# bruno-maruszczak/lap-time-optimization

Measured on AMD Instinct MI355X. Metric: MPC solves/sec (N=40, nx=8 [7 + progress s], nu=2), higher is better.
Workload: dtype f64

## Files before the change

### lap-time-optimization_amd/csrc/layout.h

```cpp
#pragma once
#include "model.h"

namespace ltompc {


constexpr int FILTER_MAX = 16;
constexpr double DW_KEEP = 1e-5;
constexpr int MAX_LS = 12;
constexpr double ELASTIC_CP_VIOL = 0.1;
constexpr double RHO_UNIT = 1000.0;
__host__ __device__ __forceinline__ double pen_scale(const double rho) { return rho > RHO_UNIT ? rho / RHO_UNIT : 1.0; }

enum : int {
  QP_A = 0,
  QP_B = 64,
  QP_b = 80,
  QP_Q = 88,
  QP_S = 124,
  QP_R = 140,
  QP_q0 = 143,
  QP_q1 = 151,
  QP_r0 = 159,
  QP_r1 = 161,
  QP_Qx = 163,
  QP_qx0 = 199,
  QP_qx1 = 207,
  QP_NF = 215
};
enum : int { RC_K = 0, RC_Kv = 16, RC_kff = 20, RC_P = 22, RC_Pxv = 58, RC_pp = 74, RC_NF = 82 };
enum : int { RS_rd = 0, RS_rp, RS_cmax, RS_cmin, RS_smult, RS_cost, RS_emax, RS_NF };
enum : int { SP_apri = 0, SP_adua, SP_gphid, SP_NF };
enum : int {
  ST_MU = 0, ST_EPS, ST_EPS_NEXT, ST_DW_LAST, ST_FORCE_REG, ST_ALPHA, ST_ADUA, ST_E0, ST_OBJ, ST_TAU,
  ST_THETA0, ST_THMAX, ST_THMIN, ST_DW, ST_DW_TRY,
  ST_C00,
  ST_RHO,
  ST_VIOL,
  ST_G0,
  ST_NF
};
enum : int { SI_STATUS = 0, SI_ITERS, SI_NACC, SI_NTINY, SI_NFILT, SI_DONE, SI_STEP, SI_NREG, SI_NLSFAIL, SI_RETRY, SI_TRIES,
             SI_SKIP_EVAL, SI_LSMORE, SI_PREV, SI_RESTO, SI_REINIT, SI_NRESTO,
             SI_STICKY,
             SI_STARTEL,
             SI_SWEEPS,
             SI_PHASE, SI_TICKS, SI_FINAL,
             SI_WARM,
             SI_SHIFT,
             SI_NSHIFT,
             SI_SINCEMU,
             SI_FBARMED,
             SI_NFALLBACK,
             SI_BLOWUP,
             SI_NODE0,
             SI_NF };

struct Work {
  int N, B, Bp;
  gptr<double> X, C, U, L1, L2, T, NU;
  gptr<double> dX, dC, dU, nL1, nL2, dT, dNU;
  gptr<double> QP, RC, RS, SP, LS;
  gptr<double> x0, uprev;
  gptr<double> st;
  gptr<double> filt;
  gptr<int> si;
  gptr<int> active;
  gptr<double> DBG;
  gptr<int> ls_list, ls_count;
  gptr<double> BK;
  gptr<const int> orig;
};

struct Launch {
  gptr<const int> act;
  gptr<const int> nact;
  int n_pad;
  int force_eval;
};

struct Consts {
  ltompc_params p;
  ltompc_options o;
  Tables T;
  Bounds bd;
};

#define PL(base, f, k, NK) ((base)[((size_t)(f) * (NK) + (k)) * W.Bp + b])
#define PG(base, f, k, NF) ((base)[(((size_t)(k) * (W.Bp >> 3) + (b >> 3)) * (NF) + (f)) * 8 + (b & 7)])


#define STD(f) st[(size_t)(f) * W.Bp + b]
#define STI(f) si[(size_t)(f) * W.Bp + b]

#define WAVE_SYNC()                                        \
  do {                                                     \
    __builtin_amdgcn_fence(__ATOMIC_RELEASE, "wavefront"); \
    __builtin_amdgcn_wave_barrier();                       \
    __builtin_amdgcn_fence(__ATOMIC_ACQUIRE, "wavefront"); \
  } while (0)

#if !defined(LTOMPC_HOST_HARNESS)
__device__ __forceinline__ double grp_max(double v) {
  v = fmax(v, __shfl_xor(v, 8)), v = fmax(v, __shfl_xor(v, 16)), v = fmax(v, __shfl_xor(v, 32));
  return v;
}
__device__ __forceinline__ double grp_sum(double v) {
  v += __shfl_xor(v, 8), v += __shfl_xor(v, 16), v += __shfl_xor(v, 32);
  return v;
}
__device__ __forceinline__ double grp_min(double v) {
  v = fmin(v, __shfl_xor(v, 8)), v = fmin(v, __shfl_xor(v, 16)), v = fmin(v, __shfl_xor(v, 32));
  return v;
}

#else
using ::grp_max;
using ::grp_min;
using ::grp_sum;
#endif

}
```

### lap-time-optimization_amd/csrc/linearise.h

```cpp
#pragma once
#include "layout.h"

namespace ltompc {

__device__ __forceinline__ double sym_get(const double* H, int i, int j) { return H[sidx(i, j)]; }


struct BoundsAny {
  static constexpr bool fixed = false;
  static constexpr unsigned ulb = 0, uub = 0, xlb = 0, xub = 0;
};
template <unsigned ULB, unsigned UUB, unsigned XLB, unsigned XUB>
struct BoundsFixed {
  static constexpr bool fixed = true;
  static constexpr unsigned ulb = ULB, uub = UUB, xlb = XLB, xub = XUB;
};
using BoundsRef = BoundsFixed<0x3, 0x3, 0xCD, 0xC4>;

template <class BP, typename F>
__device__ __forceinline__ int for_each_bound(const ltompc_params& p, F&& f) {
  int m = 0;
#pragma unroll
  for (int i = 0; i < 2; i++) {
    if (BP::fixed ? ((BP::ulb >> i) & 1u) != 0 : p.u_lb[i] > -LTOMPC_NO_BOUND) f(m++, 0, i, -1.0, p.u_lb[i]);
// ... 327 lines not shown
  if (COL < 8) {
#pragma unroll
    for (int i = 0; i <= RM; i++) v[i] = ((i == COL) ? 2.0 : 0.0) - ((COL >= elo_(i) && COL <= ehi_(i)) ? 4.0 * S.E2[i * 8 + COL] : 0.0);
  } else if (COL < 10) {
    constexpr int j = 6 + COL - 8;
#pragma unroll
    for (int i = 0; i < 8; i++) v[i] = -hdt * (((i == j) ? 1.0 : 0.0) + ((j >= elo_(i) && j <= ehi_(i)) ? 2.0 * S.E2[i * 8 + j] : 0.0));
  } else {
#pragma unroll
    for (int i = 0; i < 8; i++) {
      double s = -S.G2[i];
#pragma unroll
      for (int l = elo_(i); l <= ehi_(i); l++) s -= 2.0 * S.E2[i * 8 + l] * S.G1[l];
      v[i] = s;
    }
  }
  m8_solve<RM>(M, v, y);
#pragma unroll
  for (int i = 0; i <= RM; i++) Y[i * 11 + COL] = y[i];
#pragma unroll
  for (int i = 0; i < 8; i++) {
    double s;
    if (COL < 8) s = (i == COL) ? 2.0 : 0.0;
    else if (COL < 10) s = (i == 6 + COL - 8) ? hdt : 0.0;
    else s = S.G1[i];
#pragma unroll
    for (int l = elo_(i); l <= imin_(ehi_(i), RM); l++) s += S.E1[i * 8 + l] * y[l];
    AB[i * 11 + COL] = 2.0 * s;
  }
}

__device__ __forceinline__ bool factor_m8(const Slot& S, M8Blocks& M) {
  double maa[9], mbb[9];
#pragma unroll
  for (int i = 0; i < 6; i++)
#pragma unroll
    for (int j = gs_(i); j < 8; j++) {
      double s = (i == j) ? 4.5 : 0.0;
#pragma unroll
      for (int l = elo_(i); l <= imin_(ehi_(i), ge_(j)); l++)
        if (j >= elo_(l) && j <= ehi_(l)) s += 2.0 * S.E2[i * 8 + l] * S.E1[l * 8 + j];
      if (i < 3) {
        if (j < 3) maa[i * 3 + j] = s;
        else if (j < 6) M.ab[i * 3 + j - 3] = s;
        else M.ac[i * 2 + j - 6] = s;
      } else {
        if (j < 6) mbb[(i - 3) * 3 + j - 3] = s;
        else M.bc[(i - 3) * 2 + j - 6] = s;
      }
    }
  return inv33(maa, M.iaa) & inv33(mbb, M.ibb);
}

__device__ __forceinline__ bool condense_slot(const Consts& K, const Slot& S, M8Blocks& M, double* Y, double* AB) {
  const bool ok = factor_m8(S, M);
#pragma unroll
  for (int q = 0; q < 88; q++) Y[q] = 0.0, AB[q] = 0.0;
  condense_column<0>(K, S, M, Y, AB), condense_column<1>(K, S, M, Y, AB), condense_column<2>(K, S, M, Y, AB);
  condense_column<3>(K, S, M, Y, AB), condense_column<4>(K, S, M, Y, AB), condense_column<5>(K, S, M, Y, AB);
  condense_column<6>(K, S, M, Y, AB), condense_column<7>(K, S, M, Y, AB), condense_column<8>(K, S, M, Y, AB);
  condense_column<9>(K, S, M, Y, AB), condense_column<10>(K, S, M, Y, AB);
  return ok;
}


template <class BP, bool ELL>
__device__ __forceinline__ void d_eval(const Consts& K, const Work& W, const int k, const int b, const bool force) {
  const int N = W.N;
  if (W.si[(size_t)SI_DONE * W.Bp + b]) return;
  if (!force && (W.si[(size_t)SI_RETRY * W.Bp + b] || W.si[(size_t)SI_SKIP_EVAL * W.Bp + b])) return;
  const double hdt = K.o.t_step;
  const double eps = W.st[(size_t)ST_EPS * W.Bp + b];
  const bool reinit = W.si[(size_t)SI_REINIT * W.Bp + b] != 0;
  if (reinit) reinit_slot<BP>(K, W, k, b);
  Slot S;
  linearise_slot<true, BP, ELL>(K, W, k, b, eps, S);
#pragma unroll
  for (int i = 0; i < 36; i++) PG(W.QP, QP_Qx + i, k + 1, QP_NF) = S.Hxp[i];
#pragma unroll
  for (int i = 0; i < 8; i++) PG(W.QP, QP_qx0 + i, k + 1, QP_NF) = S.gxp0[i], PG(W.QP, QP_qx1 + i, k + 1, QP_NF) = S.gxp1[i];
  {
    double l1[8], l2[8], l1n[8], l2n[8], rd = 0.0, rp = 0.0, sm = 0.0;
    const int kn = k + 1 < N ? k + 1 : k;
    const bool nxt = k + 1 < N && !reinit;
#pragma unroll
    for (int i = 0; i < 8; i++) l1[i] = PL(W.L1, i, k, N), l2[i] = PL(W.L2, i, k, N), l1n[i] = PL(W.L1, i, kn, N), l2n[i] = PL(W.L2, i, kn, N);
#pragma unroll
    for (int a = 0; a < 8; a++) {
      double rcx = S.dcd[a] + 4.5 * l2[a];
      double rxp = S.dxd[a] - 0.5 * l1[a];
#pragma unroll
      for (int i = 0; i <= ge_(a); i++)
        if (a >= elo_(i) && a <= ehi_(i)) rcx += S.E1[i * 8 + a] * l1[i], rxp += S.E2[i * 8 + a] * l2[i];
      {
        const double t = 2.0 * l1n[a] - 2.0 * l2n[a];
        const double r2 = rxp + t;
        rxp = nxt ? r2 : rxp;
      }
      rd = fmax(rd, fmax(fabs(rcx), fabs(rxp)));
      rp = fmax(rp, fmax(fabs(S.G1[a]), fabs(S.G2[a])));
      sm += fabs(l1[a]) + fabs(l2[a]);
    }
    double cost = S.cost;
#pragma unroll
    for (int i = 0; i < 2; i++) {
      double v = k ? PL(W.U, i, k - 1, N) : W.uprev[(size_t)i * W.Bp + b];
      double du = S.u[i] - v;
      cost += K.p.r_du[i] * du * du;
      double ru = S.dud[i] + 2.0 * K.p.r_du[i] * du + hdt * (l1[6 + i] + l2[6 + i]);
      if (k + 1 < N) ru -= 2.0 * K.p.r_du[i] * (PL(W.U, i, k + 1, N) - S.u[i]);
      rd = fmax(rd, fabs(ru));
    }
    rp = fmax(rp, S.rp_ineq), sm += S.smult;
    const double cmax = S.cmax, cmin = S.cmin;
    double th0 = S.th_ineq;
#pragma unroll
    for (int a = 0; a < 8; a++) th0 += fabs(S.G1[a]) + fabs(S.G2[a]);
    PL(W.LS, 0, k, N) = th0, PL(W.LS, 1, k, N) = cost, PL(W.LS, 2, k, N) = S.sumlog;
    PL(W.RS, RS_rd, k, N) = rd, PL(W.RS, RS_rp, k, N) = rp, PL(W.RS, RS_cmax, k, N) = cmax;
    PL(W.RS, RS_cmin, k, N) = cmin, PL(W.RS, RS_smult, k, N) = sm, PL(W.RS, RS_cost, k, N) = cost;
    PL(W.RS, RS_emax, k, N) = S.emax;
  }
  M8Blocks M8;
  double Y[88], AB[88];
  condense_slot(K, S, M8, Y, AB);
#pragma unroll
  for (int i = 0; i < 8; i++) {
#pragma unroll
    for (int j = 0; j < 8; j++) PG(W.QP, QP_A + i * 8 + j, k, QP_NF) = AB[i * 11 + j];
    PG(W.QP, QP_B + i * 2 + 0, k, QP_NF) = AB[i * 11 + 8], PG(W.QP, QP_B + i * 2 + 1, k, QP_NF) = AB[i * 11 + 9];
    PG(W.QP, QP_b + i, k, QP_NF) = AB[i * 11 + 10];
  }
  double HY[88];
#pragma unroll
  for (int i = 0; i < 8; i++)
#pragma unroll
    for (int col = 0; col < 11; col++) {
      double s = 0.0;
#pragma unroll
      for (int l = 0; l <= yrow_(col); l++)
        if (hnz_(i, l)) s += sym_get(S.Hc, i, l) * Y[l * 11 + col];
      HY[i * 11 + col] = s;
    }
#pragma unroll
  for (int i = 0; i < 10; i++) {
#pragma unroll
    for (int j = 0; j < 10; j++) {
      if (j > i) continue;
      double s = 0.0;
#pragma unroll
      for (int l = 0; l <= yrow_(i); l++) s += Y[l * 11 + i] * HY[l * 11 + j];
      if (i < 8) PG(W.QP, QP_Q + sidx(i, j), k, QP_NF) = s;
      else if (j < 8) PG(W.QP, QP_S + (i - 8) * 8 + j, k, QP_NF) = s;
      else PG(W.QP, QP_R + sidx(i - 8, j - 8), k, QP_NF) = s + ((i == j) ? S.Du[i - 8] : 0.0);
    }
    double s0 = 0.0, s1 = 0.0;
#pragma unroll
    for (int l = 0; l <= yrow_(i); l++) s0 += Y[l * 11 + i] * (HY[l * 11 + 10] + S.gc0[l]), s1 += Y[l * 11 + i] * S.gc1[l];
    if (i < 8) PG(W.QP, QP_q0 + i, k, QP_NF) = s0, PG(W.QP, QP_q1 + i, k, QP_NF) = s1;
    else PG(W.QP, QP_r0 + i - 8, k, QP_NF) = s0 + S.gub0[i - 8], PG(W.QP, QP_r1 + i - 8, k, QP_NF) = s1 + S.gub1[i - 8];
  }
}

template <class BP, bool ELL>
__global__ void __launch_bounds__(64) k_eval(const Consts* __restrict__ Kp, const Work* __restrict__ Wp, Launch la) {
  const Consts& K = *Kp;
  const Work& W = *Wp;
  int tid = blockIdx.x * blockDim.x + threadIdx.x;
  int j = tid % la.n_pad, k = tid / la.n_pad;
  if (k >= W.N || j >= la.nact[0]) return;
  d_eval<BP, ELL>(K, W, k, la.act[j], la.force_eval != 0);
}


template <class BP, bool ELL>
__device__ __forceinline__ void d_expand(const Consts& K, const Work& W, const int k, const int b) {
  const int N = W.N;
  if (W.si[(size_t)SI_DONE * W.Bp + b] || !W.si[(size_t)SI_STEP * W.Bp + b]) return;
  const double mu = W.st[(size_t)ST_MU * W.Bp + b], eps = W.st[(size_t)ST_EPS * W.Bp + b];
  const double tau = W.st[(size_t)ST_TAU * W.Bp + b], rho = W.st[(size_t)ST_RHO * W.Bp + b];
  double pi[8];
  {
    double dxp0[8], du0[2];
#pragma unroll
    for (int i = 0; i < 8; i++) dxp0[i] = PL(W.dX, i, k + 1, N + 1);
    du0[0] = PL(W.dU, 0, k, N), du0[1] = PL(W.dU, 1, k, N);
#pragma unroll
    for (int i = 0; i < 8; i++) {
      double s = PG(W.RC, RC_pp + i, k + 1, RC_NF) + PG(W.RC, RC_Pxv + i * 2, k + 1, RC_NF) * du0[0] +
                 PG(W.RC, RC_Pxv + i * 2 + 1, k + 1, RC_NF) * du0[1];
#pragma unroll
      for (int j = 0; j < 8; j++) s += PG(W.RC, RC_P + sidx(i, j), k + 1, RC_NF) * dxp0[j];
      pi[i] = s;
    }
  }
  __builtin_amdgcn_sched_barrier(0);
  Slot S;
  linearise_slot<false, BP, ELL>(K, W, k, b, eps, S);
  M8Blocks M8;
  factor_m8(S, M8);
  double dxk[8], dxp[8], du[2], dc[8];
#pragma unroll
  for (int i = 0; i < 8; i++) dxk[i] = PL(W.dX, i, k, N + 1), dxp[i] = PL(W.dX, i, k + 1, N + 1);
  du[0] = PL(W.dU, 0, k, N), du[1] = PL(W.dU, 1, k, N);
  {
    const double hdt = K.o.t_step;
    double w[8], v[8];
#pragma unroll
    for (int l = 0; l < 8; l++) w[l] = 2.0 * dxk[l] + (l >= 6 ? hdt * du[l - 6] : 0.0) + S.G1[l];
#pragma unroll
    for (int i = 0; i < 8; i++) {
      double s = 2.0 * dxk[i] - (i >= 6 ? hdt * du[i - 6] : 0.0) - S.G2[i];
#pragma unroll
      for (int l = elo_(i); l <= ehi_(i); l++) s -= 2.0 * S.E2[i * 8 + l] * w[l];
      v[i] = s;
    }
    m8_solve<7>(M8, v, dc);
#pragma unroll
    for (int i = 0; i < 8; i++) PL(W.dC, i, k, N) = dc[i];
  }
  double v[8];
#pragma unroll
  for (int i = 0; i < 8; i++) {
    double s = S.gc0[i] + mu * S.gc1[i];
#pragma unroll
    for (int j = 0; j < 8; j++) {
      if (hnz_(i, j)) s += sym_get(S.Hc, i, j) * dc[j];
      if (i >= elo_(j) && i <= ehi_(j)) s += 2.0 * S.E1[j * 8 + i] * pi[j];
    }
    v[i] = -s;
  }
  {
    double l2[8];
    m8_solve_t(M8, v, l2);
#pragma unroll
    for (int i = 0; i < 8; i++) v[i] = l2[i];
  }
#pragma unroll
  for (int i = 0; i < 8; i++) {
    double s = pi[i];
#pragma unroll
    for (int j = 0; j < 8; j++)
      if (i >= elo_(j) && i <= ehi_(j)) s += S.E2[j * 8 + i] * v[j];
    PL(W.nL1, i, k, N) = 2.0 * s;
    PL(W.nL2, i, k, N) = v[i];
  }
  double r_pri = 0.0, a_dua = 1.0, gphid = 0.0;
#pragma unroll
  for (int i = 0; i < 2; i++) {
    double v0 = k ? PL(W.U, i, k - 1, N) : W.uprev[(size_t)i * W.Bp + b];
    double dv0 = k ? PL(W.dU, i, k - 1, N) : 0.0;
    gphid += 2.0 * K.p.r_du[i] * (S.u[i] - v0) * (du[i] - dv0);
  }
#pragma unroll
  for (int a = 0; a < 8; a++) gphid += S.gcost[a] * dxp[a];
  double tt[BP::fixed ? MAX_NI + 3 : 1], nn[BP::fixed ? MAX_NI : 1];
  if (BP::fixed) {
    const int m0 = for_each_bound<BP>(K.p, [&](int m, int, int, double, double) { tt[m] = PL(W.T, m, k, N), nn[m] = PL(W.NU, m, k, N); });
    if (S.nl) {
#pragma unroll
      for (int q = 0; q < 3; q++) {
        tt[m0 + q] = PL(W.T, m0 + q, k, N), nn[m0 + q] = PL(W.NU, m0 + q, k, N);
        tt[m0 + 3 + q] = rho > 0.0 ? PL(W.T, K.bd.ni + q, k, N) : 0.0;
      }
    }
  }
  for_each_bound<BP>(K.p, [&](int m, int kind, int j, double sg, double val) {
    const double xv = kind == 0 ? S.u[j] : (kind == 1 ? S.c[j] : S.xp[j]);
    const double dv = kind == 0 ? du[j] : (kind == 1 ? dc[j] : dxp[j]);
    const double t = BP::fixed ? tt[m] : PL(W.T, m, k, N), nu = BP::fixed ? nn[m] : PL(W.NU, m, k, N), it = 1.0 / t;
    const double dtt = -(sg * (xv - val) + t) - sg * dv;
    const double dn = (mu - nu * dtt) * it - nu;
    PL(W.dT, m, k, N) = dtt, PL(W.dNU, m, k, N) = dn;
    r_pri = fmax(r_pri, -dtt * it);
    if (dn < 0.0) a_dua = fmin(a_dua, -tau * nu / dn);
    gphid -= mu * dtt * it;
  });
#pragma unroll
  for (int q = 0; q < 3; q++) {
    const int m = S.m_nl + q;
    if (S.nl) {
      const double t = BP::fixed ? tt[m] : PL(W.T, m, k, N), nu = BP::fixed ? nn[m] : PL(W.NU, m, k, N), it = 1.0 / t;
      const double gd = S.gs[q] * dxp[0] + S.gn[q] * dxp[1] + S.gm[q] * dxp[2];
      if (rho > 0.0) {
        double dtt, dn, dee;
        track_soft_step(rho, mu, tau, S.gv[q], gd, t, nu, BP::fixed ? tt[m + 3] : PL(W.T, K.bd.ni + q, k, N), dtt, dn, dee, r_pri, a_dua, gphid);
        PL(W.dT, m, k, N) = dtt, PL(W.dNU, m, k, N) = dn, PL(W.dT, K.bd.ni + q, k, N) = dee;
      } else {
        const double dtt = -(S.gv[q] + t) - gd;
        const double dn = (mu - nu * dtt) * it - nu;
        PL(W.dT, m, k, N) = dtt, PL(W.dNU, m, k, N) = dn;
        r_pri = fmax(r_pri, -dtt * it);
        if (dn < 0.0) a_dua = fmin(a_dua, -tau * nu / dn);
        gphid -= mu * dtt * it;
      }
    } else {
      PL(W.dT, m, k, N) = 0.0, PL(W.dNU, m, k, N) = 0.0, PL(W.dT, K.bd.ni + q, k, N) = 0.0;
    }
  }
  if (ELL) {
#pragma unroll
    for (int q = 0; q < 2; q++) {
      const int m = S.m_nl + 3 + q, me = K.bd.ni + 3 + q;
      if (S.nl) {
        const double t = PL(W.T, m, k, N), nu = PL(W.NU, m, k, N), e = PL(W.T, me, k, N);
        double gd = 0.0;
#pragma unroll
        for (int a = 0; a < 5; a++) gd += S.ge[q][a] * dxp[3 + a];
        double dtt, dn, dee;
        track_soft_step(K.p.ell_penalty, mu, tau, S.gve[q], gd, t, nu, e, dtt, dn, dee, r_pri, a_dua, gphid);
        PL(W.dT, m, k, N) = dtt, PL(W.dNU, m, k, N) = dn, PL(W.dT, me, k, N) = dee;
      } else {
        PL(W.dT, m, k, N) = 0.0, PL(W.dNU, m, k, N) = 0.0, PL(W.dT, me, k, N) = 0.0;
      }
    }
  }
  const double a_pri = r_pri > tau ? tau / r_pri : 1.0;
  PL(W.SP, SP_apri, k, N) = a_pri, PL(W.SP, SP_adua, k, N) = a_dua, PL(W.SP, SP_gphid, k, N) = gphid;
}

template <class BP, bool ELL>
__global__ void __launch_bounds__(64) k_expand(const Consts* __restrict__ Kp, const Work* __restrict__ Wp, Launch la) {
  const Consts& K = *Kp;
  const Work& W = *Wp;
  int tid = blockIdx.x * blockDim.x + threadIdx.x;
  int j = tid % la.n_pad, k = tid / la.n_pad;
  if (k >= W.N || j >= la.nact[0]) return;
  d_expand<BP, ELL>(K, W, k, la.act[j]);
}

}
```

### lap-time-optimization_amd/csrc/ltompc.hip

```cpp
#include <hip/hip_runtime.h>

#include <algorithm>
#include <cmath>
#include <cstdio>
#include <cstdlib>
#include <cstring>
#include <string>
#include <type_traits>
#include <vector>

#include "kernels.h"

using namespace ltompc;

namespace {

thread_local std::string g_err;

int fail(const std::string& msg) {
  g_err = msg;
  return -1;
}
#define HIPCHECK(expr)                                                                         \
  do {                                                                                         \
// ... 7 lines not shown

struct ltompc_solver {
  Consts K;
  Work W;
  int device = 0, N = 0, B = 0, Bp = 0, n_table = 0, max_iter = 0;
  hipStream_t own_stream = nullptr, stream = nullptr;
  std::vector<void*> allocs;
  double* d_tables = nullptr;
  double* d_x0_rm = nullptr;
  double* d_u0_rm = nullptr;
  double* d_io = nullptr;
  int* h_active = nullptr;
  int *d_act[2] = {nullptr, nullptr}, *d_nact[2] = {nullptr, nullptr};
  int last_compactions = 0;
  int *d_perm = nullptr, *d_orig = nullptr;
  int ls_width_env = 0;
  int pack_num = 6;
  bool packed = false;
  bool packing = true;
  std::vector<int> history;
  bool cold_next = true;
  bool after_rollout = false;
  int poll_every = 4;
  int profiling = 0;
  bool compaction = true;
  bool serial_riccati = false;
  std::vector<hipEvent_t> ev, ev_pool;
  size_t ev_pool_used = 0;
  std::vector<int> ev_kind, ev_width, ev_iter;
  std::vector<int> log_kind, log_width, log_iter;
  std::vector<double> log_ms;
  int cur_width = 0;
  int cur_iter = 0;
  int* d_counts = nullptr;
  int solver_counts[8] = {};
  static constexpr int ROLL_RING = 16, ROLL_PLANTS = 4;
  int* d_roll = nullptr;
  int* d_plist = nullptr;
  hipStream_t plant_streams[ROLL_PLANTS] = {};
  int n_plant_streams = 2;
  hipEvent_t ev_fin[ROLL_RING] = {}, ev_done[ROLL_RING] = {};
  long long roll_iterations = 0, roll_launches = 0;
  double ms_by_kernel[NKERN] = {};
  int launches_by_kernel[NKERN] = {};
  Consts* d_K = nullptr;
  Work* d_W = nullptr;
  bool bounds_ref = false;
  bool ref_eval = false, ref_expand = false, ref_ls = false, ref_step1 = false;
  bool eval8 = true;
  int step1_width = 512;
  int sweeps_width = 16;
  int ric1q_width = 16;
  int ric1_width = 512;
  int last_launches = 0, last_iterations = 0;
  int sens_state = 0;
  bool sens_moved = false;
  Work Ws{};
  Work* d_Ws = nullptr;
  int *d_sens_inertia = nullptr, *d_sens_ok = nullptr;
  double *d_sens_du0 = nullptr, *d_sens_margin = nullptr, *d_sens_dX = nullptr, *d_sens_dU = nullptr;

  bool poison = false;
  template <typename P>
  int dalloc(P* p, size_t n, bool work = false) {
    using T = std::remove_pointer_t<P>;
    void* q = nullptr;
    hipError_t e = hipMalloc(&q, n * sizeof(T));
    if (e != hipSuccess) return fail(std::string("hipMalloc: ") + hipGetErrorString(e));
    e = hipMemsetAsync(q, (work && poison) ? 0xFF : 0, n * sizeof(T), stream);
    if (e != hipSuccess) return fail(std::string("hipMemset: ") + hipGetErrorString(e));
    allocs.push_back(q);
    *p = (P)q;
    return 0;
  }
};

namespace {

void build_bounds(const ltompc_params& p, Bounds& b) {
  std::memset(&b, 0, sizeof b);
  for (int i = 0; i < NX; i++) {
    if (p.x_lb[i] > -LTOMPC_NO_BOUND) b.xb_idx[b.n_xb] = i, b.xb_sgn[b.n_xb] = -1.0, b.xb_val[b.n_xb] = p.x_lb[i], b.n_xb++;
    if (p.x_ub[i] < LTOMPC_NO_BOUND) b.xb_idx[b.n_xb] = i, b.xb_sgn[b.n_xb] = +1.0, b.xb_val[b.n_xb] = p.x_ub[i], b.n_xb++;
  }
  for (int i = 0; i < NU; i++) {
    if (p.u_lb[i] > -LTOMPC_NO_BOUND) b.ub_idx[b.n_ub] = i, b.ub_sgn[b.n_ub] = -1.0, b.ub_val[b.n_ub] = p.u_lb[i], b.n_ub++;
    if (p.u_ub[i] < LTOMPC_NO_BOUND) b.ub_idx[b.n_ub] = i, b.ub_sgn[b.n_ub] = +1.0, b.ub_val[b.n_ub] = p.u_ub[i], b.n_ub++;
  }
  b.nel = p.ell_penalty > 0.0 ? NEL : 0;
  b.ni = b.n_ub + 2 * b.n_xb + NNL + b.nel;
}

struct Launcher {
  ltompc_solver* h;
  int launches = 0;
  size_t lds = 0;
  int block_threads = 64;
  int stamp(int kind) {
    if (h->ev_pool_used == h->ev_pool.size()) {
      hipEvent_t e;
      if (hipEventCreate(&e) != hipSuccess) return fail("hipEventCreate failed");
      h->ev_pool.push_back(e);
    }
    hipEvent_t e = h->ev_pool[h->ev_pool_used++];
    if (hipEventRecord(e, h->stream) != hipSuccess) return fail("hipEventRecord failed");
    h->ev.push_back(e), h->ev_kind.push_back(kind), h->ev_width.push_back(h->cur_width), h->ev_iter.push_back(h->cur_iter);
    return 0;
  }
  int close() { return (h->profiling && !h->ev_kind.empty() && h->ev_kind.back() >= 0) ? stamp(-1) : 0; }
  template <typename Kern, typename... Args>
  int run(int kind, Kern kern, int threads_total, Args... args) {
    dim3 block(block_threads), grid((threads_total + block_threads - 1) / block_threads);
    const size_t lds_bytes = lds;
    lds = 0, block_threads = 64;
    if (h->profiling == 1) {
      if (stamp(kind)) return -1;
    } else if (h->profiling >= 2) {
      if (kind == h->profiling - 2) {
        if (stamp(kind)) return -1;
      } else if (!h->ev_kind.empty() && h->ev_kind.back() >= 0 && stamp(-1)) return -1;
    }
    hipLaunchKernelGGL(kern, grid, block, lds_bytes, h->stream, args...);
    launches++;
    return 0;
  }
};

int launch_iteration(ltompc_solver* h, Launcher& L, const Launch& la, const int it, const int n_launch, const int ls_width, const bool ell,
                     const bool riccati_only) {
  const int N = h->N, np = la.n_pad;
    if (h->eval8 ? L.run(0, k_eval8, N * np * 8, h->d_K, h->d_W, la) : L.run(0, ell ? (h->ref_eval ? k_eval<BoundsRef, true> : k_eval<BoundsAny, true>) : (h->ref_eval ? k_eval<BoundsRef, false> : k_eval<BoundsAny, false>), N * np, h->d_K, h->d_W, la)) return -1;
    if (h->serial_riccati) {
      if (L.run(1, k_riccati, np, h->d_K, h->d_W, la, it)) return -1;
    } else {
      const int max_sweeps = 1;
      if (n_launch <= h->ric1_width) {
        if (n_launch <= h->ric1q_width) {
          L.lds = ric1q_lds_bytes(N), L.block_threads = 256;
          if (L.run(6, k_riccati1q, n_launch * 256, h->K, h->W, la, it, n_launch <= h->sweeps_width ? 4 : 1)) return -1;
        } else {
          L.lds = ric1_lds_bytes(N);
          if (L.run(6, k_riccati1, n_launch * 64, h->K, h->W, la, it, n_launch <= h->sweeps_width ? 4 : 1)) return -1;
        }
      } else if (L.run(1, k_riccati8, np * 8, h->K, h->W, la, it, max_sweeps)) return -1;
    }
    if (riccati_only) return 0;
    if (h->eval8 ? L.run(2, k_expand8, N * np * 8, h->d_K, h->d_W, la) : L.run(2, ell ? (h->ref_expand ? k_expand<BoundsRef, true> : k_expand<BoundsAny, true>) : (h->ref_expand ? k_expand<BoundsRef, false> : k_expand<BoundsAny, false>), N * np, h->d_K, h->d_W, la)) return -1;
    if (n_launch <= h->step1_width) {
      L.block_threads = 320;
      if (L.run(7, ell ? (h->ref_step1 ? k_step1<BoundsRef, true> : k_step1<BoundsAny, true>) : (h->ref_step1 ? k_step1<BoundsRef, false> : k_step1<BoundsAny, false>), n_launch * 320, h->d_K, h->d_W, la)) return -1;
    } else {
      const auto kls = ell ? (h->ref_ls ? k_linesearch<BoundsRef, true> : k_linesearch<BoundsAny, true>) : (h->ref_ls ? k_linesearch<BoundsRef, false> : k_linesearch<BoundsAny, false>);
      if (L.run(3, kls, N * np, h->d_K, h->d_W, la, 0, np)) return -1;
      if (L.run(4, k_pick, np * 8, h->d_K, h->d_W, la, 0)) return -1;
      if (h->K.o.n_linesearch > 1) {
        const int jw = np < ls_width ? np : ls_width;
        if (L.run(3, kls, (h->K.o.n_linesearch - 1) * N * jw, h->d_K, h->d_W, la, 1, jw)) return -1;
        if (L.run(4, k_pick, jw * 8, h->d_K, h->d_W, la, 1)) return -1;
      }
      if (L.run(5, k_update, N * np, h->d_K, h->d_W, la)) return -1;
    }
  return 0;
}

int collect_profile(ltompc_solver* h) {
  for (size_t i = 0; i + 1 < h->ev_kind.size(); i++) {
    if (h->ev_kind[i] < 0) continue;
    float ms = 0.f;
    HIPCHECK(hipEventElapsedTime(&ms, h->ev[i], h->ev[i + 1]));
    h->ms_by_kernel[h->ev_kind[i]] += ms;
    h->launches_by_kernel[h->ev_kind[i]] += 1;
    h->log_kind.push_back(h->ev_kind[i]), h->log_width.push_back(h->ev_width[i]), h->log_iter.push_back(h->ev_iter[i]), h->log_ms.push_back(ms);
  }
  h->ev.clear(), h->ev_kind.clear(), h->ev_width.clear(), h->ev_iter.clear();
  h->ev_pool_used = 0;
  return 0;
}

int planes_to_host(ltompc_solver* h, const double* dev, int F, int NK, double* out) {
  if (!out) return 0;
  std::vector<double> tmp((size_t)F * NK * h->Bp);
  HIPCHECK(hipMemcpyAsync(tmp.data(), dev, tmp.size() * sizeof(double), hipMemcpyDeviceToHost, h->stream));
  HIPCHECK(hipStreamSynchronize(h->stream));
  for (int b = 0; b < h->B; b++)
    for (int k = 0; k < NK; k++)
      for (int f = 0; f < F; f++) out[((size_t)b * NK + k) * F + f] = tmp[((size_t)f * NK + k) * h->Bp + b];
  return 0;
}


int ensure_unpacked(ltompc_solver* h) {
  if (!h->packed) return 0;
  const int B = h->B, N = h->N;
  hipLaunchKernelGGL(k_pack_inverse, dim3((B + 63) / 64), dim3(64), 0, h->stream, h->d_orig, h->d_perm, B);
  const int nthreads = (N + 1) * B;
  for (int pass = 0; pass < 2; pass++)
    hipLaunchKernelGGL(k_pack, dim3((nthreads + 255) / 256), dim3(256), 0, h->stream, h->W, h->d_perm, (const int*)nullptr, B, h->d_orig,
                       h->K.bd.ni, h->K.bd.nel, pass);
  HIPCHECK(hipGetLastError());
  h->packed = false;
// ... 114 lines not shown
  HIPCHECK(hipGetDeviceCount(&ndev));
  if (device < 0 || device >= ndev) return fail("ltompc_create: no such HIP device");
  HIPCHECK(hipSetDevice(device));
  auto* h = new ltompc_solver();
  h->device = device, h->N = n_horizon, h->B = batch, h->Bp = (batch + 63) / 64 * 64, h->n_table = n_table;
  h->max_iter = options->max_iter;
  h->K.p = *params, h->K.o = *options;
  build_bounds(*params, h->K.bd);
  if (hipStreamCreateWithFlags(&h->own_stream, hipStreamNonBlocking) != hipSuccess) {
    delete h;
    return fail("hipStreamCreate failed");
  }
  h->stream = h->own_stream;
  {
    const char* e = getenv("LTOMPC_RICCATI");
    h->serial_riccati = e && std::string(e) == "serial";
    const char* po = getenv("LTOMPC_POISON");
    h->poison = po && std::string(po) == "1";
    const char* c = getenv("LTOMPC_COMPACT");
    h->compaction = !(c && std::string(c) == "0");
    const char* pk = getenv("LTOMPC_PACK");
    h->packing = !(pk && std::string(pk) == "0");
    const char* lw = getenv("LTOMPC_LSW");
    if (lw && atoi(lw) >= 64) h->ls_width_env = atoi(lw);
    const char* pn = getenv("LTOMPC_PACK_NUM");
    if (pn && atoi(pn) >= 1 && atoi(pn) <= 7) h->pack_num = atoi(pn);
    const char* ev = getenv("LTOMPC_EVAL");
    h->eval8 = options->latency_mode == 1 || (options->latency_mode == 0 && batch <= 64);
    if (ev) h->eval8 = std::string(ev) == "wave";
    if (params->ell_penalty > 0.0) h->eval8 = false;
    {
      unsigned ulb = 0, uub = 0, xlb = 0, xub = 0;
      for (int i = 0; i < 2; i++) ulb |= (params->u_lb[i] > -LTOMPC_NO_BOUND) << i, uub |= (params->u_ub[i] < LTOMPC_NO_BOUND) << i;
      for (int i = 0; i < 8; i++) xlb |= (params->x_lb[i] > -LTOMPC_NO_BOUND) << i, xub |= (params->x_ub[i] < LTOMPC_NO_BOUND) << i;
      const char* bp = getenv("LTOMPC_BOUNDS");
      h->bounds_ref = ulb == BoundsRef::ulb && uub == BoundsRef::uub && xlb == BoundsRef::xlb && xub == BoundsRef::xub &&
                      !(bp && std::string(bp) == "any");
      const std::string sel = bp ? bp : "";
      h->ref_eval = h->bounds_ref && sel.find("eval") == std::string::npos;
      h->ref_expand = h->bounds_ref && sel.find("expand") == std::string::npos;
      h->ref_ls = h->bounds_ref && sel.find("linesearch") == std::string::npos;
      h->ref_step1 = h->bounds_ref && sel.find("step1") == std::string::npos;
    }
    const char* s1 = getenv("LTOMPC_STEP1");
    if (s1) h->step1_width = atoi(s1);
    const char* t = getenv("LTOMPC_RIC1");
    if (t) h->ric1_width = atoi(t);
    const char* npl = getenv("LTOMPC_PLANT_STREAMS");
    if (npl) h->n_plant_streams = std::min((int)ltompc_solver::ROLL_PLANTS, std::max(1, std::atoi(npl)));
    const char* sw = getenv("LTOMPC_SWEEPS_W");
    if (sw) h->sweeps_width = atoi(sw);
    const char* rq = getenv("LTOMPC_RIC1Q");
    if (rq) h->ric1q_width = atoi(rq);
    if (std::max(ric1_lds_bytes(n_horizon), ric1q_lds_bytes(n_horizon)) > 150 * 1024) h->ric1_width = 0;
    else if (hipFuncSetAttribute(reinterpret_cast<const void*>(k_riccati1), hipFuncAttributeMaxDynamicSharedMemorySize, 150 * 1024) != hipSuccess ||
             hipFuncSetAttribute(reinterpret_cast<const void*>(k_riccati1q), hipFuncAttributeMaxDynamicSharedMemorySize, 150 * 1024) != hipSuccess) {
      (void)hipGetLastError();
      h->ric1_width = 0;
    }
  }
  const size_t N = h->N, Bp = h->Bp;
  const int ni = h->K.bd.ni;
  Work& W = h->W;
  W.N = h->N, W.B = h->B, W.Bp = h->Bp;
  int rc = 0;
  rc |= h->dalloc(&h->d_tables, (size_t)LTOMPC_TABLE_ROWS * n_table);
  rc |= h->dalloc(&W.X, 8 * (N + 1) * Bp, true), rc |= h->dalloc(&W.C, 8 * N * Bp, true), rc |= h->dalloc(&W.U, 2 * N * Bp, true);
  rc |= h->dalloc(&W.L1, 8 * N * Bp, true), rc |= h->dalloc(&W.L2, 8 * N * Bp, true);
  const size_t nel = h->K.bd.nel;
  rc |= h->dalloc(&W.T, (ni + NNL + nel) * N * Bp, true), rc |= h->dalloc(&W.NU, ni * N * Bp, true);
  rc |= h->dalloc(&W.dX, 8 * (N + 1) * Bp, true), rc |= h->dalloc(&W.dC, 8 * N * Bp, true), rc |= h->dalloc(&W.dU, 2 * N * Bp, true);
  rc |= h->dalloc(&W.nL1, 8 * N * Bp, true), rc |= h->dalloc(&W.nL2, 8 * N * Bp, true);
  rc |= h->dalloc(&W.dT, (ni + NNL + nel) * N * Bp, true), rc |= h->dalloc(&W.dNU, ni * N * Bp, true);
  rc |= h->dalloc(&W.QP, (size_t)QP_NF * (N + 1) * Bp, true), rc |= h->dalloc(&W.RC, (size_t)RC_NF * (N + 1) * Bp, true);
  rc |= h->dalloc(&W.RS, (size_t)RS_NF * N * Bp, true), rc |= h->dalloc(&W.SP, (size_t)SP_NF * N * Bp, true);
  rc |= h->dalloc(&W.LS, (size_t)3 * (options->n_linesearch + 1) * N * Bp, true);
  rc |= h->dalloc(&W.x0, 8 * Bp), rc |= h->dalloc(&W.uprev, 2 * Bp);
  rc |= h->dalloc(&W.st, (size_t)ST_NF * Bp), rc |= h->dalloc(&W.filt, (size_t)2 * FILTER_MAX * Bp);
  rc |= h->dalloc(&W.si, (size_t)SI_NF * Bp), rc |= h->dalloc(&W.active, (size_t)h->max_iter + 2);
  rc |= h->dalloc(&h->d_act[0], Bp), rc |= h->dalloc(&h->d_act[1], Bp), rc |= h->dalloc(&h->d_nact[0], 4), rc |= h->dalloc(&h->d_nact[1], 4);
  rc |= h->dalloc(&W.ls_list, Bp), rc |= h->dalloc(&W.ls_count, 4);
  rc |= h->dalloc(&h->d_perm, Bp), rc |= h->dalloc(&h->d_orig, Bp);
  rc |= h->dalloc(&W.BK, 18 * N * Bp, true);
  rc |= h->dalloc(&h->d_counts, 32), rc |= h->dalloc(&h->d_roll, 2 * ltompc_solver::ROLL_RING);
  rc |= h->dalloc(&h->d_plist, (size_t)ltompc_solver::ROLL_RING * h->Bp);
  if (getenv("LTOMPC_DBG")) rc |= h->dalloc(&W.DBG, 8 * N * Bp);
  rc |= h->dalloc(&h->d_x0_rm, 8 * Bp), rc |= h->dalloc(&h->d_u0_rm, 2 * Bp), rc |= h->dalloc(&h->d_io, 32 * Bp);
  if (rc) {
    ltompc_destroy(h);
    return -1;
  }
  if (hipHostMalloc((void**)&h->h_active, sizeof(int) * 4) != hipSuccess) {
    ltompc_destroy(h);
    return fail("hipHostMalloc failed");
  }
  W.orig = (gptr<const int>)h->d_orig;
  hipLaunchKernelGGL(k_act_identity, dim3((h->B + 63) / 64), dim3(64), 0, h->stream, h->d_orig, h->d_perm, h->B);
  if (hipMemcpyAsync(h->d_tables, tables, sizeof(double) * LTOMPC_TABLE_ROWS * n_table, hipMemcpyHostToDevice, h->stream) != hipSuccess ||
      hipStreamSynchronize(h->stream) != hipSuccess) {
    ltompc_destroy(h);
    return fail("table upload failed");
  }
  Tables& T = h->K.T;
  T.n = n_table;
  using tp = gptr<const double>;
  T.s_kappa = (tp)h->d_tables, T.kappa = (tp)(h->d_tables + n_table), T.s_arc = (tp)(h->d_tables + 2 * (size_t)n_table);
  T.n_left = (tp)(h->d_tables + 3 * (size_t)n_table), T.n_right = (tp)(h->d_tables + 4 * (size_t)n_table), T.v_ref = (tp)(h->d_tables + 5 * (size_t)n_table);
  T.g0_kappa = tables[0], T.inv_kappa = (double)(n_table - 1) / (tables[n_table - 1] - tables[0]);
  T.period = options->periodic_tables ? tables[n_table - 1] - tables[0] : 0.0;
  T.g0_arc = tables[2 * (size_t)n_table], T.inv_arc = (double)(n_table - 1) / (tables[3 * (size_t)n_table - 1] - tables[2 * (size_t)n_table]);
  if (h->dalloc(&h->d_K, 1) || h->dalloc(&h->d_W, 1) ||
      hipMemcpyAsync(h->d_K, &h->K, sizeof(Consts), hipMemcpyHostToDevice, h->stream) != hipSuccess ||
      hipMemcpyAsync(h->d_W, &h->W, sizeof(Work), hipMemcpyHostToDevice, h->stream) != hipSuccess ||
      hipStreamSynchronize(h->stream) != hipSuccess) {
    ltompc_destroy(h);
    return fail("ltompc_create: upload of the constants failed");
  }
  *out = h;
  return 0;
}

int ltompc_destroy(ltompc_handle h) {
  if (!h) return 0;
  (void)hipSetDevice(h->device);
  if (h->stream) (void)hipStreamSynchronize(h->stream);
  for (void* p : h->allocs) (void)hipFree(p);
  for (hipEvent_t e : h->ev_pool) (void)hipEventDestroy(e);
  if (h->h_active) (void)hipHostFree(h->h_active);
  if (h->own_stream) (void)hipStreamDestroy(h->own_stream);
  for (auto& ps : h->plant_streams)
    if (ps) (void)hipStreamDestroy(ps);
  for (int i = 0; i < ltompc_solver::ROLL_RING; i++) {
    if (h->ev_fin[i]) (void)hipEventDestroy(h->ev_fin[i]);
    if (h->ev_done[i]) (void)hipEventDestroy(h->ev_done[i]);
  }
  delete h;
  return 0;
}

// ... 598 lines not shown
```

### lap-time-optimization_amd/csrc/sensitivity.h

```cpp
#pragma once
#include "eval8.h"
#include "linearise.h"
#include "riccati.h"

namespace ltompc {

constexpr int SENS_NP = 10;

__global__ void __launch_bounds__(64) k_sens_eval8(const Consts* __restrict__ Kp, const Work* __restrict__ Wsp) {
  const Consts& K = *Kp;
  const Work& W = *Wsp;
  __shared__ E8Lds lds[8];
  const int lane = threadIdx.x, g = lane & 7, i = lane >> 3;
  const int G8 = W.Bp >> 3;
  const int k = blockIdx.x / G8, j = (blockIdx.x % G8) * 8 + g;
  const bool valid = j < W.B;
  d_eval8(K, W, lds[g], i, k, valid ? j : 0, valid);
}

template <class BP, bool ELL>
__global__ void __launch_bounds__(64) k_sens_eval(const Consts* __restrict__ Kp, const Work* __restrict__ Wsp) {
  const Consts& K = *Kp;
  const Work& W = *Wsp;
  const int tid = blockIdx.x * blockDim.x + threadIdx.x;
  const int b = tid % W.Bp, k = tid / W.Bp;
  if (k >= W.N || b >= W.B) return;
  d_eval<BP, ELL>(K, W, k, b, true);
}

__global__ void __launch_bounds__(64) k_sens_riccati8(Consts K, Work Ws, const int* __restrict__ si_solve, int* __restrict__ inertia) {
  __shared__ RicLds L;
  const int lane = threadIdx.x, g = lane & 7, i = lane >> 3;
  const int j = blockIdx.x * 8 + g;
  const bool valid = j < Ws.B;
  const int b = valid ? j : 0;
  const size_t Bp = Ws.Bp;
  const int node0 = si_solve[(size_t)SI_NODE0 * Bp + b];
  const int status = node0 ? node0 - 1 : si_solve[(size_t)SI_STATUS * Bp + b];
  const bool el = valid && (status == LTOMPC_STATUS_SOLVED || status == LTOMPC_STATUS_ACCEPTABLE) && !si_solve[(size_t)SI_REINIT * Bp + b];
  d_riccati8<true>(K, Ws, L, g, i, b, valid, -1, 1, el, inertia);
}

__global__ void __launch_bounds__(64) k_sens_forward(Work W, const int* __restrict__ inertia, int ni, double* __restrict__ du0,
                                                     int* __restrict__ ok_out, double* __restrict__ margin, double* __restrict__ dXo,
                                                     double* __restrict__ dUo, const int* __restrict__ ok_known) {
  __shared__ double xs[8][8 * SENS_NP];
  const int lane = threadIdx.x, g = lane & 7, i = lane >> 3;
  const int j = blockIdx.x * 8 + g;
  const bool valid = j < W.B;
  const int b = valid ? j : 0;
  const int N = W.N;
  const size_t ob = W.orig[b];
  const bool okk = ok_known ? ok_known[ob] != 0 : true;
  double dx[SENS_NP], dv[2][SENS_NP], du[2][SENS_NP];
#pragma unroll
  for (int c = 0; c < SENS_NP; c++) dx[c] = (c == i) ? 1.0 : 0.0, dv[0][c] = (c == 8) ? 1.0 : 0.0, dv[1][c] = (c == 9) ? 1.0 : 0.0;
  if (valid && dXo) {
#pragma unroll
    for (int c = 0; c < SENS_NP; c++) dXo[(ob * (N + 1) * 8 + i) * SENS_NP + c] = okk ? dx[c] : 0.0;
  }
  double A[8], Bi[2], Kc[2], Kv[4];
  auto load = [&](const int k, double* a, double* bb, double* kc, double* kv) {
#pragma unroll
    for (int l = 0; l < 8; l++) a[l] = PG(W.QP, QP_A + i * 8 + l, k, QP_NF);
    bb[0] = PG(W.QP, QP_B + i * 2, k, QP_NF), bb[1] = PG(W.QP, QP_B + i * 2 + 1, k, QP_NF);
    kc[0] = PG(W.RC, RC_K + i, k, RC_NF), kc[1] = PG(W.RC, RC_K + 8 + i, k, RC_NF);
#pragma unroll
    for (int l = 0; l < 4; l++) kv[l] = PG(W.RC, RC_Kv + l, k, RC_NF);
  };
  load(0, A, Bi, Kc, Kv);
  bool fin = true;
#pragma unroll 1
  for (int k = 0; k < N; k++) {
    double An[8], Bn[2], Kcn[2], Kvn[4];
    load(k + 1 < N ? k + 1 : k, An, Bn, Kcn, Kvn);
#pragma unroll
    for (int c = 0; c < 2; c++)
#pragma unroll
      for (int col = 0; col < SENS_NP; col++)
        du[c][col] = grp_sum(Kc[c] * dx[col]) + Kv[c * 2] * dv[0][col] + Kv[c * 2 + 1] * dv[1][col];
// ... 51 lines not shown
```

Measured before the change: 152,700.

## Cache linearisation results from eval for reuse in expand kernel

Adds a LIN buffer in which the eval kernel stores linearisation quantities (constraint Jacobians, Hessian entries, cost gradients, M8 block factors). Variants of the eval and expand kernels use this buffer when the active width is small. The expand kernel then reloads these values in staged parts instead of recomputing linearise_slot and factor_m8. This trades redundant arithmetic for extra global memory traffic and a larger buffer, and skipped evals now still run a linearisation so the cache stays valid.

```diff
diff --git a/lap-time-optimization_amd/csrc/layout.h b/lap-time-optimization_amd/csrc/layout.h
--- a/lap-time-optimization_amd/csrc/layout.h
+++ b/lap-time-optimization_amd/csrc/layout.h
@@ -69,6 +69,8 @@
   gptr<int> ls_list, ls_count;
   gptr<double> BK;
   gptr<const int> orig;
+  gptr<double> LIN;
+  int LP;
 };
 
 struct Launch {
diff --git a/lap-time-optimization_amd/csrc/linearise.h b/lap-time-optimization_amd/csrc/linearise.h
--- a/lap-time-optimization_amd/csrc/linearise.h
+++ b/lap-time-optimization_amd/csrc/linearise.h
@@ -403,6 +403,57 @@
   return inv33(maa, M.iaa) & inv33(mbb, M.ibb);
 }
 
+template <int PART, bool ELL, typename F>
+__device__ __forceinline__ void for_each_lin(Slot& S, M8Blocks& M, F&& f) {
+  int q = 0;
+  auto g = [&](int part, double& v) {
+    if (PART == 0 || PART == part || (PART == 4 && part > 0) || (PART == 5 && part == 0)) f(q, v);
+    q++;
+  };
+#pragma unroll
+  for (int i = 0; i < 8; i++) g(1, S.G1[i]), g(1, S.G2[i]), g(2, S.gc0[i]), g(2, S.gc1[i]), g(3, S.gcost[i]);
+#pragma unroll
+  for (int i = 0; i < 8; i++)
+#pragma unroll
+    for (int l = elo_(i); l <= ehi_(i); l++) g(2, S.E1[i * 8 + l]), g(1, S.E2[i * 8 + l]);
+#pragma unroll
+  for (int i = 0; i < 8; i++)
+#pragma unroll
+    for (int j = 0; j <= i; j++)
+      if (hnz_(i, j)) g(2, S.Hc[sidx(i, j)]);
+#pragma unroll
+  for (int i = 0; i < 3; i++) g(3, S.gs[i]), g(3, S.gn[i]), g(3, S.gm[i]), g(3, S.gv[i]);
+  if (ELL) {
+#pragma unroll
+    for (int i = 0; i < 2; i++) {
+      g(3, S.gve[i]);
+#pragma unroll
+      for (int a = 0; a < 5; a++) g(3, S.ge[i][a]);
+    }
+  }
+  auto m = [&](double& v) {
+    if (PART == 0 || PART == 1 || PART == 5) f(q, v);
+    q++;
+  };
+#pragma unroll
+  for (int i = 0; i < 9; i++) m(M.iaa[i]), m(M.ibb[i]), m(M.ab[i]);
+#pragma unroll
+  for (int i = 0; i < 6; i++) m(M.ac[i]), m(M.bc[i]);
+}
+__host__ __device__ constexpr int lin_hnz() {
+  int n = 0;
+  for (int i = 0; i < 8; i++)
+    for (int j = 0; j <= i; j++) n += hnz_(i, j) ? 1 : 0;
+  return n;
+}
+__host__ __device__ constexpr int lin_band() {
+  int n = 0;
+  for (int i = 0; i < 8; i++) n += ehi_(i) - elo_(i) + 1;
+  return n;
+}
+__host__ __device__ constexpr int lin_nf(bool ell) { return 40 + 2 * lin_band() + lin_hnz() + 12 + (ell ? 12 : 0) + 39; }
+#define PJ(base, f, k, NK) ((base)[((size_t)(f) * (NK) + (k)) * W.LP + j])
+
 __device__ __forceinline__ bool condense_slot(const Consts& K, const Slot& S, M8Blocks& M, double* Y, double* AB) {
   const bool ok = factor_m8(S, M);
 #pragma unroll
@@ -415,17 +466,28 @@
 }
 
 
-template <class BP, bool ELL>
-__device__ __forceinline__ void d_eval(const Consts& K, const Work& W, const int k, const int b, const bool force) {
+template <class BP, bool ELL, bool LIN = false>
+__device__ __forceinline__ void d_eval(const Consts& K, const Work& W, const int k, const int b, const int j, const bool force) {
   const int N = W.N;
   if (W.si[(size_t)SI_DONE * W.Bp + b]) return;
-  if (!force && (W.si[(size_t)SI_RETRY * W.Bp + b] || W.si[(size_t)SI_SKIP_EVAL * W.Bp + b])) return;
+  const bool keep = !force && (W.si[(size_t)SI_RETRY * W.Bp + b] || W.si[(size_t)SI_SKIP_EVAL * W.Bp + b]);
+  if (keep && !LIN) return;
   const double hdt = K.o.t_step;
   const double eps = W.st[(size_t)ST_EPS * W.Bp + b];
-  const bool reinit = W.si[(size_t)SI_REINIT * W.Bp + b] != 0;
+  const bool reinit = !keep && W.si[(size_t)SI_REINIT * W.Bp + b] != 0;
   if (reinit) reinit_slot<BP>(K, W, k, b);
   Slot S;
   linearise_slot<true, BP, ELL>(K, W, k, b, eps, S);
+  if (LIN && keep) {
+    M8Blocks M8;
+    factor_m8(S, M8);
+    for_each_lin<0, ELL>(S, M8, [&](int f, double& v) { PJ(W.LIN, f, k, N) = v; });
+    return;
+  }
+  if (LIN) {
+    M8Blocks none;
+    for_each_lin<4, ELL>(S, none, [&](int f, double& v) { PJ(W.LIN, f, k, N) = v; });
+  }
 #pragma unroll
   for (int i = 0; i < 36; i++) PG(W.QP, QP_Qx + i, k + 1, QP_NF) = S.Hxp[i];
 #pragma unroll
@@ -475,6 +537,7 @@
   M8Blocks M8;
   double Y[88], AB[88];
   condense_slot(K, S, M8, Y, AB);
+  if (LIN) for_each_lin<5, ELL>(S, M8, [&](int f, double& v) { PJ(W.LIN, f, k, N) = v; });
 #pragma unroll
   for (int i = 0; i < 8; i++) {
 #pragma unroll
@@ -520,12 +583,21 @@
   int tid = blockIdx.x * blockDim.x + threadIdx.x;
   int j = tid % la.n_pad, k = tid / la.n_pad;
   if (k >= W.N || j >= la.nact[0]) return;
-  d_eval<BP, ELL>(K, W, k, la.act[j], la.force_eval != 0);
-}
-
-
+  d_eval<BP, ELL>(K, W, k, la.act[j], j, la.force_eval != 0);
+}
 template <class BP, bool ELL>
-__device__ __forceinline__ void d_expand(const Consts& K, const Work& W, const int k, const int b) {
+__global__ void __launch_bounds__(64) k_eval_lin(const Consts* __restrict__ Kp, const Work* __restrict__ Wp, Launch la) {
+  const Consts& K = *Kp;
+  const Work& W = *Wp;
+  int tid = blockIdx.x * blockDim.x + threadIdx.x;
+  int j = tid % la.n_pad, k = tid / la.n_pad;
+  if (k >= W.N || j >= la.nact[0]) return;
+  d_eval<BP, ELL, true>(K, W, k, la.act[j], j, la.force_eval != 0);
+}
+
+
+template <class BP, bool ELL, bool LIN = false>
+__device__ __forceinline__ void d_expand(const Consts& K, const Work& W, const int k, const int b, const int j) {
   const int N = W.N;
   if (W.si[(size_t)SI_DONE * W.Bp + b] || !W.si[(size_t)SI_STEP * W.Bp + b]) return;
   const double mu = W.st[(size_t)ST_MU * W.Bp + b], eps = W.st[(size_t)ST_EPS * W.Bp + b];
@@ -547,9 +619,18 @@
   }
   __builtin_amdgcn_sched_barrier(0);
   Slot S;
-  linearise_slot<false, BP, ELL>(K, W, k, b, eps, S);
   M8Blocks M8;
-  factor_m8(S, M8);
+  if (LIN) {
+#pragma unroll
+    for (int i = 0; i < 8; i++) S.xp[i] = PL(W.X, i, k + 1, N + 1), S.c[i] = PL(W.C, i, k, N);
+    S.u[0] = PL(W.U, 0, k, N), S.u[1] = PL(W.U, 1, k, N);
+    for_each_lin<1, ELL>(S, M8, [&](int f, double& v) { v = PJ(W.LIN, f, k, N); });
+    S.m_nl = for_each_bound<BP>(K.p, [](int, int, int, double, double) {});
+    S.nl = (k + 1 <= N - 1);
+  } else {
+    linearise_slot<false, BP, ELL>(K, W, k, b, eps, S);
+    factor_m8(S, M8);
+  }
   double dxk[8], dxp[8], du[2], dc[8];
 #pragma unroll
   for (int i = 0; i < 8; i++) dxk[i] = PL(W.dX, i, k, N + 1), dxp[i] = PL(W.dX, i, k + 1, N + 1);
@@ -570,6 +651,10 @@
 #pragma unroll
     for (int i = 0; i < 8; i++) PL(W.dC, i, k, N) = dc[i];
   }
+  if (LIN) {
+    __builtin_amdgcn_sched_barrier(0);
+    for_each_lin<2, ELL>(S, M8, [&](int f, double& v) { v = PJ(W.LIN, f, k, N); });
+  }
   double v[8];
 #pragma unroll
   for (int i = 0; i < 8; i++) {
@@ -595,6 +680,10 @@
       if (i >= elo_(j) && i <= ehi_(j)) s += S.E2[j * 8 + i] * v[j];
     PL(W.nL1, i, k, N) = 2.0 * s;
     PL(W.nL2, i, k, N) = v[i];
+  }
+  if (LIN) {
+    __builtin_amdgcn_sched_barrier(0);
+    for_each_lin<3, ELL>(S, M8, [&](int f, double& v) { v = PJ(W.LIN, f, k, N); });
   }
   double r_pri = 0.0, a_dua = 1.0, gphid = 0.0;
 #pragma unroll
@@ -677,7 +766,16 @@
   int tid = blockIdx.x * blockDim.x + threadIdx.x;
   int j = tid % la.n_pad, k = tid / la.n_pad;
   if (k >= W.N || j >= la.nact[0]) return;
-  d_expand<BP, ELL>(K, W, k, la.act[j]);
-}
-
-}
+  d_expand<BP, ELL>(K, W, k, la.act[j], j);
+}
+template <class BP, bool ELL>
+__global__ void __launch_bounds__(64) k_expand_lin(const Consts* __restrict__ Kp, const Work* __restrict__ Wp, Launch la) {
+  const Consts& K = *Kp;
+  const Work& W = *Wp;
+  int tid = blockIdx.x * blockDim.x + threadIdx.x;
+  int j = tid % la.n_pad, k = tid / la.n_pad;
+  if (k >= W.N || j >= la.nact[0]) return;
+  d_expand<BP, ELL, true>(K, W, k, la.act[j], j);
+}
+
+}
diff --git a/lap-time-optimization_amd/csrc/ltompc.hip b/lap-time-optimization_amd/csrc/ltompc.hip
--- a/lap-time-optimization_amd/csrc/ltompc.hip
+++ b/lap-time-optimization_amd/csrc/ltompc.hip
@@ -83,6 +83,7 @@
   int sweeps_width = 16;
   int ric1q_width = 16;
   int ric1_width = 512;
+  int expand_lin_width = -1;
   int last_launches = 0, last_iterations = 0;
   int sens_state = 0;
   bool sens_moved = false;
@@ -160,7 +161,10 @@
 int launch_iteration(ltompc_solver* h, Launcher& L, const Launch& la, const int it, const int n_launch, const int ls_width, const bool ell,
                      const bool riccati_only) {
   const int N = h->N, np = la.n_pad;
-    if (h->eval8 ? L.run(0, k_eval8, N * np * 8, h->d_K, h->d_W, la) : L.run(0, ell ? (h->ref_eval ? k_eval<BoundsRef, true> : k_eval<BoundsAny, true>) : (h->ref_eval ? k_eval<BoundsRef, false> : k_eval<BoundsAny, false>), N * np, h->d_K, h->d_W, la)) return -1;
+  const bool lin = !h->eval8 && np <= h->W.LP && n_launch <= (h->expand_lin_width >= 0 ? h->expand_lin_width : h->ric1_width);
+    if (lin) {
+      if (L.run(0, ell ? (h->ref_eval ? k_eval_lin<BoundsRef, true> : k_eval_lin<BoundsAny, true>) : (h->ref_eval ? k_eval_lin<BoundsRef, false> : k_eval_lin<BoundsAny, false>), N * np, h->d_K, h->d_W, la)) return -1;
+    } else if (h->eval8 ? L.run(0, k_eval8, N * np * 8, h->d_K, h->d_W, la) : L.run(0, ell ? (h->ref_eval ? k_eval<BoundsRef, true> : k_eval<BoundsAny, true>) : (h->ref_eval ? k_eval<BoundsRef, false> : k_eval<BoundsAny, false>), N * np, h->d_K, h->d_W, la)) return -1;
     if (h->serial_riccati) {
       if (L.run(1, k_riccati, np, h->d_K, h->d_W, la, it)) return -1;
     } else {
@@ -176,7 +180,9 @@
       } else if (L.run(1, k_riccati8, np * 8, h->K, h->W, la, it, max_sweeps)) return -1;
     }
     if (riccati_only) return 0;
-    if (h->eval8 ? L.run(2, k_expand8, N * np * 8, h->d_K, h->d_W, la) : L.run(2, ell ? (h->ref_expand ? k_expand<BoundsRef, true> : k_expand<BoundsAny, true>) : (h->ref_expand ? k_expand<BoundsRef, false> : k_expand<BoundsAny, false>), N * np, h->d_K, h->d_W, la)) return -1;
+    if (lin) {
+      if (L.run(2, ell ? (h->ref_expand ? k_expand_lin<BoundsRef, true> : k_expand_lin<BoundsAny, true>) : (h->ref_expand ? k_expand_lin<BoundsRef, false> : k_expand_lin<BoundsAny, false>), N * np, h->d_K, h->d_W, la)) return -1;
+    } else if (h->eval8 ? L.run(2, k_expand8, N * np * 8, h->d_K, h->d_W, la) : L.run(2, ell ? (h->ref_expand ? k_expand<BoundsRef, true> : k_expand<BoundsAny, true>) : (h->ref_expand ? k_expand<BoundsRef, false> : k_expand<BoundsAny, false>), N * np, h->d_K, h->d_W, la)) return -1;
     if (n_launch <= h->step1_width) {
       L.block_threads = 320;
       if (L.run(7, ell ? (h->ref_step1 ? k_step1<BoundsRef, true> : k_step1<BoundsAny, true>) : (h->ref_step1 ? k_step1<BoundsRef, false> : k_step1<BoundsAny, false>), n_launch * 320, h->d_K, h->d_W, la)) return -1;
@@ -397,6 +403,8 @@
     if (sw) h->sweeps_width = atoi(sw);
     const char* rq = getenv("LTOMPC_RIC1Q");
     if (rq) h->ric1q_width = atoi(rq);
+    const char* el = getenv("LTOMPC_EXPAND_LIN");
+    if (el) h->expand_lin_width = std::max(0, atoi(el));
     if (std::max(ric1_lds_bytes(n_horizon), ric1q_lds_bytes(n_horizon)) > 150 * 1024) h->ric1_width = 0;
     else if (hipFuncSetAttribute(reinterpret_cast<const void*>(k_riccati1), hipFuncAttributeMaxDynamicSharedMemorySize, 150 * 1024) != hipSuccess ||
              hipFuncSetAttribute(reinterpret_cast<const void*>(k_riccati1q), hipFuncAttributeMaxDynamicSharedMemorySize, 150 * 1024) != hipSuccess) {
@@ -430,6 +438,11 @@
   rc |= h->dalloc(&h->d_counts, 32), rc |= h->dalloc(&h->d_roll, 2 * ltompc_solver::ROLL_RING);
   rc |= h->dalloc(&h->d_plist, (size_t)ltompc_solver::ROLL_RING * h->Bp);
   if (getenv("LTOMPC_DBG")) rc |= h->dalloc(&W.DBG, 8 * N * Bp);
+  {
+    const int lw = std::min((int)Bp, h->expand_lin_width >= 0 ? h->expand_lin_width : (h->ric1_width > 0 ? 512 : 0));
+    W.LP = h->eval8 ? 0 : (lw + 63) / 64 * 64;
+    if (W.LP) rc |= h->dalloc(&W.LIN, (size_t)lin_nf(nel > 0) * N * W.LP, true);
+  }
   rc |= h->dalloc(&h->d_x0_rm, 8 * Bp), rc |= h->dalloc(&h->d_u0_rm, 2 * Bp), rc |= h->dalloc(&h->d_io, 32 * Bp);
   if (rc) {
     ltompc_destroy(h);
diff --git a/lap-time-optimization_amd/csrc/sensitivity.h b/lap-time-optimization_amd/csrc/sensitivity.h
--- a/lap-time-optimization_amd/csrc/sensitivity.h
+++ b/lap-time-optimization_amd/csrc/sensitivity.h
@@ -25,7 +25,7 @@
   const int tid = blockIdx.x * blockDim.x + threadIdx.x;
   const int b = tid % W.Bp, k = tid / W.Bp;
   if (k >= W.N || b >= W.B) return;
-  d_eval<BP, ELL>(K, W, k, b, true);
+  d_eval<BP, ELL>(K, W, k, b, 0, true);
 }
 
 __global__ void __launch_bounds__(64) k_sens_riccati8(Consts K, Work Ws, const int* __restrict__ si_solve, int* __restrict__ inertia) {
diff --git a/profiles/r05/summarize_trace.py b/profiles/r05/summarize_trace.py
--- /dev/null
+++ b/profiles/r05/summarize_trace.py
@@ -0,0 +1,25 @@
+import csv, glob, json, sys
+from collections import defaultdict
+
+src, out_prefix, N = sys.argv[1], sys.argv[2], 40
+files = glob.glob(f"{src}/**/*kernel_trace.csv", recursive=True)
+tot, cnt, split = defaultdict(float), defaultdict(int), defaultdict(lambda: [0, 0.0])
+for f in files:
+    with open(f) as fh:
+        for r in csv.DictReader(fh):
+            name = r["Kernel_Name"]
+            us = (int(r["End_Timestamp"]) - int(r["Start_Timestamp"])) / 1000.0
+            tot[name] += us; cnt[name] += 1
+            g = int(r.get("Grid_Size_X") or r.get("Grid_Size") or 0)
+            short = name.split("(")[0].replace("void ", "").replace("ltompc::", "")
+            if short.startswith(("k_eval", "k_expand")):
+                key = short + (" narrow" if g <= 128 * N else " wide")
+                split[key][0] += 1; split[key][1] += us
+all_us = sum(tot.values())
+with open(out_prefix + "_kernel_stats.csv", "w") as fh:
+    fh.write("kernel,calls,avg_us,total_ms,percent\n")
+    for name in sorted(tot, key=lambda n: -tot[n]):
+        fh.write(f"\"{name}\",{cnt[name]},{tot[name] / cnt[name]:.1f},{tot[name] / 1000:.3f},{100 * tot[name] / all_us:.2f}\n")
+with open(out_prefix + "_eval_expand_split.json", "w") as fh:
+    json.dump({k: {"launches": v[0], "mean_us": round(v[1] / v[0], 2), "total_ms": round(v[1] / 1000, 3)} for k, v in sorted(split.items())}, fh, indent=1)
+print(open(out_prefix + "_eval_expand_split.json").read())
```

After: 154,700, median of 6. Within noise of the previous version (+1.3%).
